# rfahrn/RadVLM

Hardware: AMD Instinct MI355X
Metric: train image-instruction pairs/sec, LLaVA-1.5-7B 336px (higher is better)
Workload: dtype bf16; 1 GPU; llava15_7b full fine-tune step (ViT frozen): fwd+bwd+AdamW, S=704, 32 pairs/GPU/step; global_batch=32, seq_len=704, parallelism=dp1, rows_with_a_label_only=last layer's o_proj / norm / MLP, final norm, lm_head, cross entropy

## Files before the change

include/radvlm_hip.h:

```cpp
#ifndef RADVLM_HIP_H
#define RADVLM_HIP_H
#include <stdint.h>

#ifdef __cplusplus
extern "C" {
#endif

#define RV_ACT_NONE 0
#define RV_ACT_QUICK_GELU 1
#define RV_ACT_GELU 2
#define RV_ACT_GELU_TANH 3

const char* rv_version(void);

int rv_gemm_nt_bf16(const void* A, int64_t lda, const void* B, int64_t ldb, void* C, int64_t ldc, const void* bias,
                    const void* residual, int64_t ldr, int M, int N, int K, int act, int out_f32, int res_f32,
                    const void* zeros16, void* stream);
int rv_gemm_bf16(const void* A, int64_t lda, const void* B, int64_t ldb, void* C, int64_t ldc, const void* bias,
                 const void* residual, int64_t ldr, int M, int N, int K, int trans_a, int trans_b, float alpha, int act,
                 int out_f32, int res_f32, const void* zeros16, void* stream);
int rv_gemm_bf16_ex(const void* A, int64_t lda, const void* B, int64_t ldb, void* C, int64_t ldc, const void* bias,
                    const void* residual, int64_t ldr, int M, int N, int K, int trans_a, int trans_b, float alpha, int act,
                    int out_f32, int res_f32, const void* A2, int64_t lda2, const void* B2, int64_t ldb2, int K2,
                    void* workspace, int64_t workspace_bytes, const void* zeros16, void* stream);
int rv_gemm_rope_bf16(const void* A, int64_t lda, const void* B, int64_t ldb, void* C, int64_t ldc, const void* bias, int M, int N, int K,
                      const float* cos_sin, const int32_t* positions, int S, int rope_heads, int hd, void* workspace,
                      int64_t workspace_bytes, const void* zeros16, void* stream);
int rv_gemm_swiglu_fwd_bf16(const void* A, int64_t lda, const void* Wgu, int64_t ldb, void* GU, int64_t ldgu, void* ACT, int64_t ldact,
                            int M, int F, int K, void* workspace, int64_t workspace_bytes, const void* zeros16, void* stream);
int rv_gemm_swiglu_bwd_bf16(const void* dY, int64_t ldy, const void* Wd, int64_t ldw, const void* GU, int64_t ldgu, void* dGU, int64_t lddgu,
                            void* dact_scratch, int64_t ld_dact, int M, int F, int K, void* workspace, int64_t workspace_bytes,
                            const void* zeros16, void* stream);
int rv_gemm_select_kernel(int which);
int rv_gemm_set_cu_budget(int total_cus, int reserved_cus);

int rv_transpose_bf16(const void* in, int64_t in_ld, int64_t in_bs0, int64_t in_bs1, void* out, int64_t out_ld,
                      int64_t out_bs0, int64_t out_bs1, int R, int C, int R_pad, int nb0, int nb1, int perm32,
                      void* stream);

int rv_rmsnorm_fwd(const void* x, const void* w, void* y, float* rstd, int rows, int d, float eps, void* stream);
int rv_rmsnorm_bwd(const void* dy, const void* x, const void* w, const float* rstd, void* dx, int dx_add,
                   float* dw_partial, int nblk, int rows, int d, void* stream);
int rv_layernorm_fwd(const void* x, const void* w, const void* b, void* y, float* stats, int rows, int d, float eps,
                     void* stream);
int rv_layernorm_bwd(const void* dy, const void* x, const void* w, const float* stats, void* dx, int dx_add,
                     float* partial, int nblk, int rows, int d, void* stream);
int rv_quick_gelu_fwd(const void* x, void* y, int64_t n, void* stream);
int rv_quick_gelu_bwd(const void* dy, const void* x, void* dx, int64_t n, void* stream);

int rv_gelu_tanh_fwd(const void* x, void* y, int64_t n, void* stream);
int rv_gelu_tanh_bwd(const void* dy, const void* x, void* dx, int64_t n, void* stream);

int rv_colsum_f32(const float* in, int rows, int cols, void* out_bf16, int accumulate, void* stream);
int rv_colsum_partial_bf16(const void* x, int64_t ld, int rows, int cols, float* partial, int nblk, void* stream);

int rv_rope_inplace(void* x, int64_t ld, const float* cos_sin, int rows, int S, int heads, int hd, int nsec, int dir,
                    void* stream);

int rv_attn_fwd(const void* q, int64_t ld_q, const void* k, int64_t ld_k, const void* vT, void* out, int64_t ld_o,
                float* lse, const int32_t* lens, int B, int H, int S, int S_pad, int hd, int causal, float scale,
                const void* zeros16, void* stream);
int rv_attn_bwd(const void* q, int64_t ld_q, const void* k, int64_t ld_k, const void* v, int64_t ld_v, const void* o,
                int64_t ld_o, const void* dout, int64_t ld_do, const void* qT, const void* kT, const void* doT,
                const float* lse, float* delta, void* dq, int64_t ld_dq, void* dk, int64_t ld_dk, void* dv,
                int64_t ld_dv, const int32_t* lens, int B, int H, int S, int S_pad, int hd, int causal, float scale,
                const void* zeros16, void* stream);

int rv_attn_fwd_gqa(const void* q, int64_t ld_q, const void* k, int64_t ld_k, const void* vT, void* out, int64_t ld_o,
                    float* lse, const int32_t* lens, const int32_t* cu_rows, int B, int H, int H_kv, int S, int S_pad, int hd,
                    int causal, float scale, const void* zeros16, void* stream);
int rv_attn_fwd_nat(const void* q, int64_t ld_q, const void* k, int64_t ld_k, const void* v, int64_t ld_v, void* out, int64_t ld_o,
                    float* lse, const int32_t* lens, const int32_t* cu_rows, int B, int H, int H_kv, int S, int S_pad, int hd, int causal,
                    float scale, const void* zeros16, void* stream);
int rv_attn_fwd_nat_pairs(int B, int H, int S, int causal);
int rv_attn_bwd_gqa(const void* q, int64_t ld_q, const void* k, int64_t ld_k, const void* v, int64_t ld_v, const void* o,
                    int64_t ld_o, const void* dout, int64_t ld_do, const void* qT, const void* kT, const void* doT,
                    const float* lse, float* delta, void* dq, int64_t ld_dq, void* dk, int64_t ld_dk, void* dv,
                    int64_t ld_dv, const int32_t* lens, const int32_t* cu_rows, int total_rows, int B, int H, int H_kv, int S,
                    int S_pad, int hd, int causal, float scale, void* workspace, int64_t workspace_bytes, const void* zeros16,
                    void* stream);
int rv_attn_bwd_gqa_rope(const void* q, int64_t ld_q, const void* k, int64_t ld_k, const void* v, int64_t ld_v, const void* o,
                         int64_t ld_o, const void* dout, int64_t ld_do, const void* qT, const void* kT, const void* doT,
                         const float* lse, float* delta, void* dq, int64_t ld_dq, void* dk, int64_t ld_dk, void* dv,
                         int64_t ld_dv, const int32_t* lens, const int32_t* cu_rows, int total_rows, int B, int H, int H_kv, int S,
                         int S_pad, int hd, int causal, float scale, void* workspace, int64_t workspace_bytes,
                         const float* rope_cos_sin, const int32_t* rope_positions, const void* zeros16, void* stream);

// ... 92 lines not shown
```

radvlm_amd/csrc/gemm_bf16.hip:

```cpp
#include <type_traits>
#include "common.h"
#include "radvlm_hip.h"
#include <stdlib.h>

namespace {

constexpr int BM = 128, BN = 128, BK = 64;
constexpr int STAGE_BYTES = (BM + BN) * BK * 2;
constexpr int NSTAGE = 2;

struct GemmParams {
    const bf16* A; const bf16* B; void* C; const bf16* bias; const void* R; const bf16* zeros;
    long lda, ldb, ldc, ldr;
    int M, N, K, act, out_f32, res_f32, tiles_m, tiles_n;
    float alpha;
    const bf16* A2; const bf16* B2; long lda2, ldb2; int K2;
    float* ws; int splits;
    int n_full;
    int pgrid;
    const float* rope_cs; const int* rope_pos; int rope_S, rope_cols, rope_hd;
    int F; bf16* C2; long ldc2; const bf16* G; long ldg;
    unsigned bytesA, bytesB;
    unsigned bytesA2, bytesB2;
    unsigned drop_thr; float drop_scale; unsigned long long drop_seed;
};
enum { EPI_NONE = 0, EPI_ROPE = 1, EPI_SWIGLU_FWD = 2, EPI_SWIGLU_BWD = 3 };

DEVINL float erf_as(float x) {
    const float ax = fabsf(x);
    const float t = __frcp_rn(1.f + 0.3275911f * ax);
    const float p = t * (0.254829592f + t * (-0.284496736f + t * (1.421413741f + t * (-1.453152027f + t * 1.061405429f))));
    const float r = 1.f - p * __expf(-ax * ax);
    return copysignf(r, x);
}
DEVINL float apply_act(float x, int act) {
    if (act == RV_ACT_QUICK_GELU) return x / (1.f + __expf(-1.702f * x));
    if (act == RV_ACT_GELU) return 0.5f * x * (1.f + erf_as(x * 0.70710678118654752f));
    if (act == RV_ACT_GELU_TANH) return x / (1.f + __expf(-1.5957691216057308f * (x + 0.044715f * x * x * x)));
    return x;
}

DEVINL void stage_tile(const bf16* __restrict__ src, long ld, int row0, int nrows_total, int k0, int K,
                       const bf16* zeros, char* lds, int wid, int lane) {
#pragma unroll
    for (int it = 0; it < 4; ++it) {
        const int c = (it * 4 + wid) * 64 + lane;
        const int r = c >> 3, p = c & 7;
        const int lc = p ^ ((r >> 1) & 7);
        const int gr = row0 + r, gk = k0 + lc * 8;
        const bf16* g = (gr < nrows_total && gk < K) ? (src + (long)gr * ld + gk) : zeros;
        glds16(g, lds + (it * 4 + wid) * 1024);
    }
}

DEVINL bf16x8 read_frag(const char* tile, int row, int kchunk) {
    const int p = kchunk ^ ((row >> 1) & 7);
    return *(const bf16x8*)(tile + row * 128 + p * 16);
}

__global__ __launch_bounds__(256, 2) void gemm_nt_kernel(GemmParams P) {
    extern __shared__ __attribute__((aligned(16))) char smem[];
    const int wid = wave_id(), lane = lane_id();
    const int wr = wid >> 1, wc = wid & 1;

    const int nwg = P.tiles_m * P.tiles_n;
    int pid = xcd_remap(blockIdx.x, nwg);
    constexpr int GROUP_M = 8;
    const int per_group = GROUP_M * P.tiles_n;
    const int group = pid / per_group;
    const int first_m = group * GROUP_M;
    const int gsz = min(P.tiles_m - first_m, GROUP_M);
    const int tm = first_m + (pid % per_group) % gsz;
    const int tn = (pid % per_group) / gsz;
    const int m0 = tm * BM, n0 = tn * BN;

    f32x4 acc[4][4];
#pragma unroll
    for (int i = 0; i < 4; ++i)
#pragma unroll
// ... 591 lines not shown
            bf16x8 gq[2][4], uq[2][4];
            auto fetch = [&](int bi, bf16x8 (&gd)[4], bf16x8 (&ud)[4]) {
#pragma unroll
                for (int u = 0; u < 4; ++u) {
                    const int ia = bi * 4 + u, i = ia >> 1, a = ia & 1;
                    const bf16* p = gp + (long)i * 16 * P.ldg + 32 * a;
                    gd[u] = *(const bf16x8*)p;
                    ud[u] = *(const bf16x8*)(p + P.F);
                }
            };
            fetch(0, gq[0], uq[0]);
            static_for<4>([&](auto bt) {
                constexpr int bi = decltype(bt)::value;
                if constexpr (bi + 1 < 4) fetch(bi + 1, gq[(bi + 1) & 1], uq[(bi + 1) & 1]);
                static_for<4>([&](auto ut) {
                    constexpr int u = decltype(ut)::value, ia = bi * 4 + u, i = ia >> 1, a = ia & 1;
                    bf16* c = cp + (long)i * 16 * P.ldc + 32 * a;
                    dswiglu(acc[i][2 * a], acc[i][2 * a + 1], gq[bi & 1][u], uq[bi & 1][u], c, c + P.F);
                });
            });
            return;
        }
        static_for<16>([&](auto ia) {
            constexpr int i = decltype(ia)::value >> 1, a = decltype(ia)::value & 1;
            const int m = m0 + wr * 128 + i * 16 + (lane & 15);
            const int n = tn * BN2 + wc * 64 + 32 * a + 8 * q;
            if (m >= P.M || n >= P.F) return;
            const bf16x8 gv = *(const bf16x8*)(P.G + (long)m * P.ldg + n), uv = *(const bf16x8*)(P.G + (long)m * P.ldg + P.F + n);
            bf16* cp = (bf16*)P.C + (long)m * P.ldc;
            dswiglu(acc[i][2 * a], acc[i][2 * a + 1], gv, uv, cp + n, cp + P.F + n);
        });
    }
}

#ifdef RV_STAMPS
static long long* g_stamp_host = nullptr;
extern "C" int rv_debug_set_stamp_buffer(void* p) { g_stamp_host = (long long*)p; return 0; }
#define RV_STAMP(i) do { if (MODE == 0 && P.ws && threadIdx.x == 0) ((long long*)P.ws)[(long)blockIdx.x * 4 + (i)] = wall_clock64(); } while (0)
#else
#define RV_STAMP(i) do { } while (0)
#endif

template <bool TA, bool TB, int MODE, int EPI = EPI_NONE, bool BUF = false>
__global__ __launch_bounds__(512, 1) void gemm_kernel_256(GemmParams P) {
    extern __shared__ __attribute__((aligned(16))) char smem[];
    const int wid = wave_id(), lane = lane_id();
    const int wr = wid >> 2, wc = wid & 3;
    RV_STAMP(0);

    const int nwg = P.tiles_m * P.tiles_n;
    constexpr bool PERSIST = (MODE == 0 || MODE == 1 || MODE == 3) && BUF;
    int vtile = blockIdx.x, kslice = 0;
    bool sliced = MODE == 2;
    if (MODE == 2) { vtile = (int)blockIdx.x / P.splits; kslice = (int)blockIdx.x % P.splits; }
    if (MODE == 3 && (int)blockIdx.x >= (PERSIST ? P.pgrid : P.n_full)) {
        const int r = (int)blockIdx.x - (PERSIST ? P.pgrid : P.n_full);
        vtile = P.n_full + r / P.splits; kslice = r % P.splits; sliced = true;
    }
    int m0, n0, tn;
    auto coords = [&](int vt) {
        const int pid = xcd_remap(vt, nwg);
        constexpr int GROUP_M = RV_GROUP_M;
        const int per_group = GROUP_M * P.tiles_n;
        const int group = pid / per_group;
        const int first_m = group * GROUP_M;
        const int gsz = min(P.tiles_m - first_m, GROUP_M);
        tn = (pid % per_group) / gsz;
        m0 = (first_m + (pid % per_group) % gsz) * BM2;
        n0 = tn * BN2;
    };
    coords(vtile);

    f32x4 acc[8][4];

    const int nt1 = (P.K + BK - 1) / BK;
    const int t0 = sliced ? (int)((long)kslice * nt1 / P.splits) : 0;
    const int nt = sliced ? (int)((long)(kslice + 1) * nt1 / P.splits) - t0 : (MODE == 1 ? nt1 + (P.K2 + BK - 1) / BK : nt1);
    __amdgpu_buffer_rsrc_t rsA, rsB;
    HalfPlan plA[2], plB[2];
    if constexpr (BUF) {
        rsA = __builtin_amdgcn_make_buffer_rsrc((void*)P.A, 0, P.bytesA, 0x00020000);
        rsB = __builtin_amdgcn_make_buffer_rsrc((void*)P.B, 0, P.bytesB, 0x00020000);
    }
    auto make_plans = [&]() {
#pragma unroll
        for (int h = 0; h < 2; ++h) {
            plA[h] = plan_half<TA, false, 0>(P.lda, m0 + h * 128, P.M, wid, lane, h, 0, P.bytesA);
            if (EPI == EPI_ROPE) plB[h] = P.rope_hd == 128 ? plan_half<TB, true, 1>(P.ldb, n0 + h * 128, P.N, wid, lane, h, 0, P.bytesB)
                                                            : plan_half<TB, true, 0>(P.ldb, n0 + h * 128, P.N, wid, lane, h, 0, P.bytesB);
            else if (EPI == EPI_SWIGLU_FWD) plB[h] = plan_half<TB, true, 2>(P.ldb, tn * 128, P.N, wid, lane, h, P.F, P.bytesB);
            else plB[h] = plan_half<TB, true, 0>(P.ldb, n0 + h * 128, P.N, wid, lane, h, 0, P.bytesB);
        }
    };
    __amdgpu_buffer_rsrc_t rsA2, rsB2;
    HalfPlan plA2[2], plB2[2];
    if constexpr (BUF && MODE == 1) {
        rsA2 = __builtin_amdgcn_make_buffer_rsrc((void*)P.A2, 0, P.bytesA2, 0x00020000);
        rsB2 = __builtin_amdgcn_make_buffer_rsrc((void*)P.B2, 0, P.bytesB2, 0x00020000);
    }
    auto make_plans2 = [&]() {
#pragma unroll
        for (int h = 0; h < 2; ++h) {
            plA2[h] = plan_half<TA, false, 0>(P.lda2, m0 + h * 128, P.M, wid, lane, h, 0, P.bytesA2);
            plB2[h] = plan_half<TB, true, 0>(P.ldb2, n0 + h * 128, P.N, wid, lane, h, 0, P.bytesB2);
        }
    };
    if constexpr (BUF) make_plans();
    if constexpr (BUF && MODE == 1) make_plans2();
    const int kstepA = TA ? (int)(P.lda * BK * 2) : BK * 2, kstepB = TB ? (int)(P.ldb * BK * 2) : BK * 2;
    const int kstepA2 = TA ? (int)(P.lda2 * BK * 2) : BK * 2, kstepB2 = TB ? (int)(P.ldb2 * BK * 2) : BK * 2;
    auto stageA = [&](int t, int slot, int h, auto pair_tag) {
        constexpr int PAIR = decltype(pair_tag)::value;
        char* dst = smem + (slot * 2 + h) * HALF_BYTES;
        if constexpr (BUF) {
            if (MODE == 1 && (PAIR == 1 || (PAIR == 2 && t >= nt1))) stage_half_buf(rsA2, plA2[h], (t - nt1) * kstepA2, dst, wid);
            else stage_half_buf(rsA, plA[h], (t0 + t) * kstepA, dst, wid);
            return;
        }
        if (MODE == 1 && t >= nt1) stage_half<TA>(P.A2, P.lda2, m0 + h * 128, P.M, (t - nt1) * BK, P.K2, P.zeros, dst, wid, lane);
        else stage_half<TA>(P.A, P.lda, m0 + h * 128, P.M, (t0 + t) * BK, P.K, P.zeros, dst, wid, lane);
    };
    auto stageB = [&](int t, int h, auto pair_tag) {
        constexpr int PAIR = decltype(pair_tag)::value;
        char* dst = smem + B_RING_OFF + ((t & 1) * 2 + h) * HALF_BYTES;
        if constexpr (BUF) {
            if (MODE == 1 && (PAIR == 1 || (PAIR == 2 && t >= nt1))) stage_half_buf(rsB2, plB2[h], (t - nt1) * kstepB2, dst, wid);
            else stage_half_buf(rsB, plB[h], (t0 + t) * kstepB, dst, wid);
            return;
        }
        if (MODE == 1 && t >= nt1) stage_half<TB, true>(P.B2, P.ldb2, n0 + h * 128, P.N, (t - nt1) * BK, P.K2, P.zeros, dst, wid, lane);
// ... 11 lines not shown
    int vt0 = blockIdx.x;
    do {
    if (nt > 1) { stageA(1, 1, 0, PR); stageA(1, 1, 1, PR); stageB(1, 0, PR); stageB(1, 1, PR); asm volatile("s_waitcnt vmcnt(8)" ::: "memory"); }
    else asm volatile("s_waitcnt vmcnt(0)" ::: "memory");
    __builtin_amdgcn_s_barrier();
    RV_STAMP(1);
#pragma unroll
    for (int i = 0; i < 8; ++i)
#pragma unroll
        for (int j = 0; j < 4; ++j) acc[i][j] = f32x4{0.f, 0.f, 0.f, 0.f};

    int aslot = 0;
    long long dbg[4] = {0, 0, 0, 0};
    auto step = [&](int t, auto stage_tag, auto pair_tag) {
        constexpr int STAGE = decltype(stage_tag)::value;
        const char* At = smem + (aslot * 2 + wr) * HALF_BYTES;
        const char* Bt = smem + B_RING_OFF + ((t & 1) * 2 + (wc >> 1)) * HALF_BYTES;
        const int aslot2 = aslot == 0 ? 2 : aslot - 1;
        const int brow0 = (wc & 1) * 64;
        ktile_256<TA, TB>(acc, At, Bt, brow0, lane,
                          [&]() { if (STAGE == 1 || (STAGE == 2 && t + 2 < nt)) stageA(t + 2, aslot2, 0, pair_tag); },
                          [&]() { if (STAGE == 1 || (STAGE == 2 && t + 2 < nt)) stageA(t + 2, aslot2, 1, pair_tag); },
                          [&]() { if (STAGE == 1 || (STAGE == 2 && t + 2 < nt)) stageB(t + 2, 0, pair_tag); },
                          [&]() { if (STAGE == 1 || (STAGE == 2 && t + 2 < nt)) stageB(t + 2, 1, pair_tag); }, dbg);
        RV_ACC_BEGIN();
        if (STAGE == 1 || (STAGE == 2 && t + 2 < nt)) asm volatile("s_waitcnt vmcnt(8)" ::: "memory");
        else asm volatile("s_waitcnt vmcnt(0)" ::: "memory");
        RV_ACC_END(1);
        aslot = aslot == 2 ? 0 : aslot + 1;
        RV_ACC_BEGIN();
        BAR_LGKM();
        RV_ACC_END(2);
    };
    if constexpr ((MODE == 2 || MODE == 1) && !BUF) {
        for (int t = 0; t < nt; ++t) step(t, std::integral_constant<int, 2>{}, PR);
    } else if constexpr (MODE == 1) {
        int t = 0;
        for (; t + 2 < nt1; ++t) step(t, std::integral_constant<int, 1>{}, P0);
        for (; t + 2 < nt; ++t) step(t, std::integral_constant<int, 1>{}, P1);
        for (; t < nt; ++t) step(t, std::integral_constant<int, 0>{}, P0);
    } else {
        int t = 0;
        for (; t + 2 < nt; ++t) step(t, std::integral_constant<int, 1>{}, P0);
        for (; t < nt; ++t) step(t, std::integral_constant<int, 0>{}, P0);
    }
#ifdef RV_STAMPS
    if (MODE == 0 && P.ws && lane == 0) {
        long long* o = (long long*)P.ws + (long)gridDim.x * 4 + ((long)blockIdx.x * 8 + wid) * 3;
        o[0] = dbg[0]; o[1] = dbg[1]; o[2] = dbg[2];
    }
#endif

    RV_STAMP(2);
    if (MODE == 3 && sliced) {
        float* slab = P.ws + ((long)(vtile - P.n_full) * P.splits + kslice) * (BM2 * BN2);
#pragma unroll
        for (int i = 0; i < 8; ++i)
#pragma unroll
            for (int a = 0; a < 2; ++a) {
                float* wp = slab + (wr * 128 + i * 16 + (lane & 15)) * BN2 + wc * 64 + 32 * a + 8 * (lane >> 4);
                *(f32x4*)wp = acc[i][2 * a];
                *(f32x4*)(wp + 4) = acc[i][2 * a + 1];
            }
        return;
    }
    const int m0e = m0, n0e = n0, tne = tn;
    bool more = false;
    if constexpr (PERSIST) {
        vt0 += MODE == 3 ? P.pgrid : (int)gridDim.x;
        more = !sliced && vt0 < (MODE == 3 ? P.n_full : nwg);
        if (more) {
            coords(vt0); make_plans();
            if constexpr (MODE == 1) make_plans2();
            stageA(0, 0, 0, P0); stageA(0, 0, 1, P0); stageB(0, 0, P0); stageB(0, 1, P0);
        }
    }
    if (EPI != EPI_NONE) epilogue_fused<EPI>(acc, P, m0e, tne, wr, wc, lane);
    else epilogue_256<MODE == 3 ? 0 : MODE>(acc, P, m0e, n0e, wr, wc, lane, kslice);
#ifdef RV_STAMPS
    asm volatile("s_waitcnt vmcnt(0)" ::: "memory");
#endif
    RV_STAMP(3);
    if (!more) break;
    } while (PERSIST);
}

__global__ void splitk_reduce_kernel(GemmParams P) {
    const long i = (long)blockIdx.x * blockDim.x + threadIdx.x;
    const long total = (long)P.M * P.N;
    if (i >= total) return;
    const int m = (int)(i / P.N), n = (int)(i % P.N);
    float s = 0.f;
    for (int k = 0; k < P.splits; ++k) s += P.ws[(long)k * total + i];
    s *= P.alpha;
    if (P.bias) s += bf2f(P.bias[n]);
    s = apply_act(s, P.act);
    if (P.R) s += P.res_f32 ? ((const float*)P.R)[(long)m * P.ldr + n] : bf2f(((const bf16*)P.R)[(long)m * P.ldr + n]);
    if (P.out_f32) ((float*)P.C)[(long)m * P.ldc + n] = s;
    else ((bf16*)P.C)[(long)m * P.ldc + n] = f2bf(s);
}

constexpr int AG_BM = 64, AG_BN = 128;
constexpr int AG_XB = AG_BM * AG_BN * 2, AG_TB = AG_BM * 64 * 2, AG_STAGE = AG_XB + AG_TB;
struct LoraAGradParams {
    const bf16* X; const bf16* T; float* ws;
    long ldx, ldt;
    int M, R, K, splits;
    unsigned thr; unsigned long long seed;
};
DEVINL int sw128(int m) { return (((m >> 1) & 1) | (((m >> 3) & 1) << 1)) << 1; }
DEVINL bf16x8 tr_read16(const char* a, const char* b) {
    const s16x4 lo = __builtin_amdgcn_ds_read_tr16_b64_v4i16((__attribute__((address_space(3))) s16x4*)a);
    const s16x4 hi = __builtin_amdgcn_ds_read_tr16_b64_v4i16((__attribute__((address_space(3))) s16x4*)b);
    const s16x8 r = {lo[0], lo[1], lo[2], lo[3], hi[0], hi[1], hi[2], hi[3]};
    return __builtin_bit_cast(bf16x8, r);
}
__global__ __launch_bounds__(256, 3) void lora_agrad_kernel(LoraAGradParams P) {
    __shared__ __attribute__((aligned(16))) char smem[2 * AG_STAGE];
    const int wid = wave_id(), lane = lane_id(), tid = (int)threadIdx.x;
    const int ncb = (P.K + AG_BN - 1) / AG_BN;
    const int cb = (int)blockIdx.x % ncb, split = (int)blockIdx.x / ncb;
// ... 34 lines not shown
#pragma unroll
    for (int i = 0; i < 4; ++i) toff[i] = AG_XB + mrow * 128 + ((((16 * i) >> 3) + (pp >> 1)) ^ sw128(mrow)) * 16 + (pp & 1) * 8;
    f32x4 acc[4][2];
#pragma unroll
    for (int i = 0; i < 4; ++i)
#pragma unroll
        for (int j = 0; j < 2; ++j) acc[i][j] = f32x4{0.f, 0.f, 0.f, 0.f};
    if (s0 < s1) { load(s0); store(s0, smem); }
    __syncthreads();
    for (int s = s0; s < s1; ++s) {
        const char* cur = smem + ((s - s0) & 1) * AG_STAGE;
        char* nxt = smem + (((s - s0) & 1) ^ 1) * AG_STAGE;
        if (s + 1 < s1) load(s + 1);
#pragma unroll
        for (int kk = 0; kk < 2; ++kk) {
            bf16x8 b[2], a[4];
#pragma unroll
            for (int j = 0; j < 2; ++j) b[j] = tr_read16(cur + xoff[j] + kk * 8192, cur + xoff[j] + kk * 8192 + 1024);
#pragma unroll
            for (int i = 0; i < 4; ++i) a[i] = tr_read16(cur + toff[i] + kk * 4096, cur + toff[i] + kk * 4096 + 512);
#pragma unroll
            for (int i = 0; i < 4; ++i)
#pragma unroll
                for (int j = 0; j < 2; ++j) acc[i][j] = mfma16(a[i], b[j], acc[i][j]);
        }
        if (s + 1 < s1) store(s + 1, nxt);
        __syncthreads();
    }
#pragma unroll
    for (int i = 0; i < 4; ++i)
#pragma unroll
        for (int j = 0; j < 2; ++j)
#pragma unroll
            for (int r = 0; r < 4; ++r) {
                const int ar = 16 * i + 4 * g + r, col = c0 + wid * 32 + 16 * j + (lane & 15);
                if (ar < P.R && col < P.K) P.ws[((long)split * P.R + ar) * P.K + col] = acc[i][j][r];
            }
}

__global__ __launch_bounds__(256) void tail_reduce_kernel(GemmParams P) {
    const int nwg = P.tiles_m * P.tiles_n;
    const int tt = blockIdx.x >> 5;
    const int e = ((blockIdx.x & 31) * 256 + threadIdx.x) * 8;
    const int row = e >> 8, col = e & 255;
    const int pid = xcd_remap(P.n_full + tt, nwg);
    constexpr int GROUP_M = RV_GROUP_M;
    const int per_group = GROUP_M * P.tiles_n;
    const int group = pid / per_group;
    const int first_m = group * GROUP_M;
    const int gsz = min(P.tiles_m - first_m, GROUP_M);
    const int m = (first_m + (pid % per_group) % gsz) * BM2 + row;
    const int n = ((pid % per_group) / gsz) * BN2 + col;
    if (m >= P.M || n >= P.N) return;
    float v[8] = {0, 0, 0, 0, 0, 0, 0, 0};
    for (int k = 0; k < P.splits; ++k) {
        const float* sp = P.ws + ((long)tt * P.splits + k) * (BM2 * BN2) + row * BN2 + col;
        const f32x4 a = *(const f32x4*)sp, b = *(const f32x4*)(sp + 4);
#pragma unroll
        for (int r = 0; r < 4; ++r) { v[r] += a[r]; v[4 + r] += b[r]; }
    }
    const int nv = min(8, P.N - n);
    const bool vec = nv == 8 && (P.N % 8 == 0) && (P.ldc % 8 == 0) && !P.out_f32 && (!P.R || (!P.res_f32 && P.ldr % 8 == 0)) &&
                     ((((uintptr_t)P.C) | ((uintptr_t)P.R) | ((uintptr_t)P.bias)) & 15) == 0;
    if (vec) {
        float x[8];
#pragma unroll
        for (int r = 0; r < 8; ++r) x[r] = v[r] * P.alpha;
        if (P.bias) {
            const bf16x8 bb = *(const bf16x8*)(P.bias + n);
#pragma unroll
            for (int r = 0; r < 8; ++r) x[r] += bf2f(bb[r]);
        }
        if (P.act != RV_ACT_NONE) {
#pragma unroll
            for (int r = 0; r < 8; ++r) x[r] = apply_act(x[r], P.act);
        }
        if (P.R) {
            const bf16x8 rr = *(const bf16x8*)((const bf16*)P.R + (long)m * P.ldr + n);
#pragma unroll
            for (int r = 0; r < 8; ++r) x[r] += bf2f(rr[r]);
        }
        *(bf16x8*)((bf16*)P.C + (long)m * P.ldc + n) = bf16x8{f2bf(x[0]), f2bf(x[1]), f2bf(x[2]), f2bf(x[3]), f2bf(x[4]), f2bf(x[5]), f2bf(x[6]), f2bf(x[7])};
        return;
    }
    for (int r = 0; r < nv; ++r) {
        float x = v[r] * P.alpha;
        if (P.bias) x += bf2f(P.bias[n + r]);
        x = apply_act(x, P.act);
        if (P.R) x += P.res_f32 ? ((const float*)P.R)[(long)m * P.ldr + n + r] : bf2f(((const bf16*)P.R)[(long)m * P.ldr + n + r]);
        if (P.out_f32) ((float*)P.C)[(long)m * P.ldc + n + r] = x;
        else ((bf16*)P.C)[(long)m * P.ldc + n + r] = f2bf(x);
    }
}

}

static int g_tail_split = 1;
static int g_force_kernel = 0;
static int g_cus = 0;
static int g_cus_device = -1;
static int g_reserved_cus = -1;
static int g_no_buf = 0;
static int g_persist = 1;
extern "C" int rv_gemm_select_kernel(int which) {
    if (which >= 40) { g_persist = which == 41; return RV_OK; }
    if (which >= 30) { g_no_buf = which == 30; return RV_OK; }
    if (which >= 20) { g_tail_split = which - 20; return RV_OK; }
    g_force_kernel = which;
    return RV_OK;
}
extern "C" int rv_gemm_set_cu_budget(int total_cus, int reserved_cus) {
    int dev = 0;
    if (hipGetDevice(&dev) != hipSuccess) return RV_ERR_LAUNCH;
    if (total_cus <= 0) {
        int n = 0;
        if (hipDeviceGetAttribute(&n, hipDeviceAttributeMultiprocessorCount, dev) != hipSuccess) return RV_ERR_LAUNCH;
        total_cus = n;
    }
    g_cus_device = dev;
    if (reserved_cus < 0) reserved_cus = 0;
    g_reserved_cus = reserved_cus;
    g_cus = total_cus - reserved_cus;
    if (g_cus < 8) g_cus = 8;
    return g_cus;
}
static int cu_budget() {
    int dev = 0;
    if (g_cus != 0 && hipGetDevice(&dev) == hipSuccess && dev != g_cus_device) g_cus = 0;
    if (g_cus == 0) {
        const char* e = getenv("RV_GEMM_RESERVED_CUS");
        rv_gemm_set_cu_budget(0, g_reserved_cus >= 0 ? g_reserved_cus : (e ? atoi(e) : 0));
    }
    return g_cus;
}

static bool buf_extents(GemmParams& P, int trans_a, int trans_b) {
    if ((P.K % BK) && !(trans_a && trans_b)) return false;
    const long ea = (trans_a ? (long)P.K : (long)P.M) * P.lda * 2, eb = (trans_b ? (long)P.K : (long)P.N) * P.ldb * 2;
    if (ea >= (1L << 31) || eb >= (1L << 31) || g_no_buf) return false;
    P.bytesA = (unsigned)ea; P.bytesB = (unsigned)eb;
    return true;
}
static bool buf_extents2(GemmParams& P, int trans_a, int trans_b) {
    if ((P.K2 % BK) && !(trans_a && trans_b)) return false;
    const long ea = (trans_a ? (long)P.K2 : (long)P.M) * P.lda2 * 2, eb = (trans_b ? (long)P.K2 : (long)P.N) * P.ldb2 * 2;
    if (ea >= (1L << 31) || eb >= (1L << 31)) return false;
    P.bytesA2 = (unsigned)ea; P.bytesB2 = (unsigned)eb;
    return true;
}
template <bool TA, bool TB, int MODE, bool BUF = false>
static void launch256m(const GemmParams& P, hipStream_t st) {
    static bool set = false;
    if (!set) { (void)hipFuncSetAttribute((const void*)gemm_kernel_256<TA, TB, MODE, EPI_NONE, BUF>, hipFuncAttributeMaxDynamicSharedMemorySize, LDS_BYTES2); set = true; }
    const int nwg = P.tiles_m * P.tiles_n;
    const int blocks = MODE == 2 ? nwg * P.splits : (MODE == 3 ? P.n_full + (nwg - P.n_full) * P.splits : nwg);
    int grid = blocks;
    GemmParams Q = P;
    Q.pgrid = MODE == 3 ? P.n_full : blocks;
    if (g_persist && BUF && (MODE == 0 || MODE == 1) && blocks > cu_budget()) { grid = cu_budget(); Q.pgrid = grid; }
    if (g_persist && BUF && MODE == 3 && P.n_full > cu_budget()) { Q.pgrid = cu_budget(); grid = Q.pgrid + (nwg - P.n_full) * P.splits; }
    hipLaunchKernelGGL((gemm_kernel_256<TA, TB, MODE, EPI_NONE, BUF>), dim3(grid), dim3(512), LDS_BYTES2, st, Q);
    if (MODE == 3) hipLaunchKernelGGL(tail_reduce_kernel, dim3((nwg - P.n_full) * 32), dim3(256), 0, st, P);
    if (MODE == 2) {
        const long total = (long)P.M * P.N;
        hipLaunchKernelGGL(splitk_reduce_kernel, dim3((unsigned)((total + 255) / 256)), dim3(256), 0, st, P);
    }
}
template <bool TA, bool TB>
static void launch256(GemmParams& P, int mode, hipStream_t st) {
    if (mode == 1) { if (buf_extents(P, TA, TB) && buf_extents2(P, TA, TB)) launch256m<TA, TB, 1, true>(P, st); else launch256m<TA, TB, 1>(P, st); }
    else if (mode == 2) { if (buf_extents(P, TA, TB)) launch256m<TA, TB, 2, true>(P, st); else launch256m<TA, TB, 2>(P, st); }
    else if (buf_extents(P, TA, TB)) { if (mode == 3) launch256m<TA, TB, 3, true>(P, st); else launch256m<TA, TB, 0, true>(P, st); }
    else if (mode == 3) launch256m<TA, TB, 3>(P, st);
    else launch256m<TA, TB, 0>(P, st);
}

static int gemm_ex_impl(const void* A, int64_t lda, const void* B, int64_t ldb, void* C, int64_t ldc, const void* bias,
                        const void* residual, int64_t ldr, int M, int N, int K, int trans_a, int trans_b, float alpha,
                        int act, int out_f32, int res_f32, const void* A2, int64_t lda2, const void* B2, int64_t ldb2,
                        int K2, void* workspace, int64_t workspace_bytes, const void* zeros16, void* stream, float drop_p, uint64_t drop_seed) {
    if (!A || !B || !C || !zeros16 || M <= 0 || N <= 0 || K <= 0) return RV_ERR_ARG;
    if ((lda & 7) || (ldb & 7)) return RV_ERR_ARG;
    if ((!trans_a && (K & 7)) || (trans_a && (M & 7)) || (!trans_b && (K & 7)) || (trans_b && (N & 7))) return RV_ERR_ARG;
    if (((uintptr_t)A | (uintptr_t)B | (uintptr_t)zeros16) & 15) return RV_ERR_ARG;
    const bool ext = A2 && B2 && K2 > 0;
    if (ext && ((lda2 & 7) || (ldb2 & 7) || (!trans_a && (K2 & 7)) || (!trans_b && (K2 & 7)) || (((uintptr_t)A2 | (uintptr_t)B2) & 15))) return RV_ERR_ARG;
    GemmParams P;
    P.A = (const bf16*)A; P.B = (const bf16*)B; P.C = C; P.bias = (const bf16*)bias; P.R = residual;
    P.zeros = (const bf16*)zeros16;
    P.lda = lda; P.ldb = ldb; P.ldc = ldc; P.ldr = ldr;
    P.M = M; P.N = N; P.K = K; P.act = act; P.out_f32 = out_f32; P.res_f32 = res_f32; P.alpha = alpha;
    P.A2 = (const bf16*)A2; P.B2 = (const bf16*)B2; P.lda2 = lda2; P.ldb2 = ldb2; P.K2 = ext ? K2 : 0;
    P.ws = (float*)workspace; P.splits = 1;
    P.drop_thr = drop_p > 0.f ? rv_dropout_thr16(drop_p) : 0u; P.drop_scale = drop_p > 0.f ? 1.f / (1.f - drop_p) : 1.f; P.drop_seed = drop_seed;
    const bool dropping = P.drop_thr != 0;
    static bool attr_set = false;
    if (!attr_set) {
        (void)hipFuncSetAttribute((const void*)gemm_nt_kernel, hipFuncAttributeMaxDynamicSharedMemorySize, NSTAGE * STAGE_BYTES);
        const char* e = getenv("RV_GEMM_KERNEL");
        if (e) g_force_kernel = atoi(e);
        attr_set = true;
    }
    const long tiles256 = (long)((M + BM2 - 1) / BM2) * ((N + BN2 - 1) / BN2);
    const int nt = (K + BK - 1) / BK;
    const int force = g_force_kernel;
    const int cus = cu_budget();
    int mode = ext ? 1 : 0;
    if (dropping) workspace = nullptr;
    if (!ext && workspace && tiles256 <= cus / 4 && nt >= 16) {
        int sp = (int)(cus / tiles256);
        if (sp > nt / 4) sp = nt / 4;
        if (sp > 32) sp = 32;
        if (sp >= 2 && (int64_t)sp * M * N * 4 <= workspace_bytes) { mode = 2; P.splits = sp; }
    }
    P.n_full = 0;
    if (mode == 0 && workspace && g_tail_split && tiles256 > cus) {
        const int rem = (int)(tiles256 % cus);
        if (rem > 0 && rem <= cus / 2 && nt >= 32) {
            int sp = cus / rem;
            if (sp > 4) sp = 4;
            if ((int64_t)rem * sp * BM2 * BN2 * 4 <= workspace_bytes) { mode = 3; P.splits = sp; P.n_full = (int)(tiles256 - rem); }
        }
    }
    const long tiles128 = (long)((M + BM - 1) / BM) * ((N + BN - 1) / BN);
    const double cost256 = 4.0 * (double)((tiles256 + cus - 1) / cus);
    const double cost128 = 2.0 * 1.15 * (double)((tiles128 + 2 * cus - 1) / (2 * cus));
    const bool use256 = (trans_a || trans_b || mode || dropping) ? true : (force ? (force == 2) : (cost256 <= cost128));
    hipStream_t st = (hipStream_t)stream;
    if (use256) {
#ifdef RV_STAMPS
        if (mode == 0) P.ws = (float*)g_stamp_host;
#endif
        P.tiles_m = (M + BM2 - 1) / BM2; P.tiles_n = (N + BN2 - 1) / BN2;
        if (trans_a) { if (trans_b) launch256<true, true>(P, mode, st); else launch256<true, false>(P, mode, st); }
        else { if (trans_b) launch256<false, true>(P, mode, st); else launch256<false, false>(P, mode, st); }
    } else {
        P.tiles_m = (M + BM - 1) / BM; P.tiles_n = (N + BN - 1) / BN;
        hipLaunchKernelGGL(gemm_nt_kernel, dim3(P.tiles_m * P.tiles_n), dim3(256), NSTAGE * STAGE_BYTES, st, P);
    }
    return rv_check_launch();
}

extern "C" int rv_gemm_bf16_ex(const void* A, int64_t lda, const void* B, int64_t ldb, void* C, int64_t ldc, const void* bias,
                               const void* residual, int64_t ldr, int M, int N, int K, int trans_a, int trans_b, float alpha,
                               int act, int out_f32, int res_f32, const void* A2, int64_t lda2, const void* B2, int64_t ldb2,
                               int K2, void* workspace, int64_t workspace_bytes, const void* zeros16, void* stream) {
    return gemm_ex_impl(A, lda, B, ldb, C, ldc, bias, residual, ldr, M, N, K, trans_a, trans_b, alpha, act, out_f32, res_f32, A2, lda2, B2, ldb2, K2,
                        workspace, workspace_bytes, zeros16, stream, 0.f, 0);
}

extern "C" int rv_gemm_dropout_add_bf16(const void* A, int64_t lda, const void* B, int64_t ldb, void* C, int64_t ldc, int M, int N, int K,
                                        int trans_b, float alpha, float p, uint64_t seed, int accumulate, const void* zeros16, void* stream) {
    if (p < 0.f || p >= 1.f || (N & 7) || (ldc & 7) || (((uintptr_t)C) & 15)) return RV_ERR_ARG;
    return gemm_ex_impl(A, lda, B, ldb, C, ldc, nullptr, accumulate ? C : nullptr, ldc, M, N, K, 0, trans_b, alpha, RV_ACT_NONE, 0, 0, nullptr, 0,
                        nullptr, 0, 0, nullptr, 0, zeros16, stream, p, seed);
}

extern "C" int rv_gemm_bf16(const void* A, int64_t lda, const void* B, int64_t ldb, void* C, int64_t ldc, const void* bias,
                            const void* residual, int64_t ldr, int M, int N, int K, int trans_a, int trans_b, float alpha,
                            int act, int out_f32, int res_f32, const void* zeros16, void* stream) {
    return rv_gemm_bf16_ex(A, lda, B, ldb, C, ldc, bias, residual, ldr, M, N, K, trans_a, trans_b, alpha, act, out_f32, res_f32,
                           nullptr, 0, nullptr, 0, 0, nullptr, 0, zeros16, stream);
}

extern "C" int rv_gemm_nt_bf16(const void* A, int64_t lda, const void* B, int64_t ldb, void* C, int64_t ldc,
                               const void* bias, const void* residual, int64_t ldr, int M, int N, int K, int act,
                               int out_f32, int res_f32, const void* zeros16, void* stream) {
    return rv_gemm_bf16(A, lda, B, ldb, C, ldc, bias, residual, ldr, M, N, K, 0, 0, 1.0f, act, out_f32, res_f32, zeros16, stream);
}

template <int EPI, bool TB, bool BUF>
static void launch_fused1(const GemmParams& P, hipStream_t st) {
    static bool attr = false;
    if (!attr) { (void)hipFuncSetAttribute((const void*)gemm_kernel_256<false, TB, 0, EPI, BUF>, hipFuncAttributeMaxDynamicSharedMemorySize, LDS_BYTES2); attr = true; }
    int grid = P.tiles_m * P.tiles_n;
// ... 123 lines not shown
```

radvlm_amd/lib.py:

```python
import ctypes
import os

import torch

_HERE = os.path.dirname(os.path.abspath(__file__))
_LIB_PATH = os.path.join(_HERE, "libradvlm_hip.so")

_c_void_p = ctypes.c_void_p
_i64 = ctypes.c_int64
_i32 = ctypes.c_int
_f32 = ctypes.c_float

ACT_NONE, ACT_QUICK_GELU, ACT_GELU, ACT_GELU_TANH = 0, 1, 2, 3

_SIGS = {
    "rv_gemm_nt_bf16": [_c_void_p, _i64, _c_void_p, _i64, _c_void_p, _i64, _c_void_p, _c_void_p, _i64, _i32, _i32, _i32,
                        _i32, _i32, _i32, _c_void_p, _c_void_p],
    "rv_gemm_bf16": [_c_void_p, _i64, _c_void_p, _i64, _c_void_p, _i64, _c_void_p, _c_void_p, _i64, _i32, _i32, _i32, _i32, _i32,
                     _f32, _i32, _i32, _i32, _c_void_p, _c_void_p],
    "rv_gemm_bf16_ex": [_c_void_p, _i64, _c_void_p, _i64, _c_void_p, _i64, _c_void_p, _c_void_p, _i64, _i32, _i32, _i32, _i32, _i32,
                        _f32, _i32, _i32, _i32, _c_void_p, _i64, _c_void_p, _i64, _i32, _c_void_p, _i64, _c_void_p, _c_void_p],
    "rv_gemm_rope_bf16": [_c_void_p, _i64, _c_void_p, _i64, _c_void_p, _i64, _c_void_p, _i32, _i32, _i32, _c_void_p, _c_void_p, _i32, _i32, _i32,
                          _c_void_p, _i64, _c_void_p, _c_void_p],
    "rv_gemm_swiglu_fwd_bf16": [_c_void_p, _i64, _c_void_p, _i64, _c_void_p, _i64, _c_void_p, _i64, _i32, _i32, _i32, _c_void_p, _i64, _c_void_p,
# ... 32 lines not shown
                        _c_void_p, _i64, _c_void_p, _i64, _c_void_p, _c_void_p, _i32, _i32, _i32, _i32, _i32, _i32, _i32, _i32, _f32, _c_void_p, _i64,
                        _c_void_p, _c_void_p, _c_void_p, _c_void_p],
    "rv_attn_bwd_gqa_rope": [_c_void_p, _i64, _c_void_p, _i64, _c_void_p, _i64, _c_void_p, _i64, _c_void_p, _i64, _c_void_p, _c_void_p,
                             _c_void_p, _c_void_p, _c_void_p, _c_void_p, _i64, _c_void_p, _i64, _c_void_p, _i64, _c_void_p, _c_void_p, _i32,
                             _i32, _i32, _i32, _i32, _i32, _i32, _i32, _f32, _c_void_p, _i64, _c_void_p, _c_void_p, _c_void_p, _c_void_p],
    "rv_transpose_bf16_varlen": [_c_void_p, _i64, _c_void_p, _i64, _c_void_p, _i64, _i64, _i64, _i32, _i32, _i32, _i32, _i32, _i32,
                                 _c_void_p],
    "rv_rope_inplace_pos": [_c_void_p, _i64, _c_void_p, _c_void_p, _i32, _i32, _i32, _i32, _i32, _c_void_p],
    "rv_gelu_tanh_fwd": [_c_void_p, _c_void_p, _i64, _c_void_p],
    "rv_gelu_tanh_bwd": [_c_void_p, _c_void_p, _c_void_p, _i64, _c_void_p],
    "rv_weighted_segment_sum_rows": [_c_void_p, _i64, _c_void_p, _c_void_p, _c_void_p, _c_void_p, _i32, _c_void_p, _i64, _i32,
                                     _c_void_p],
    "rv_max4_rows_fwd": [_c_void_p, _i64, _c_void_p, _c_void_p, _i32, _c_void_p, _i64, _c_void_p, _i32, _c_void_p],
    "rv_max4_rows_bwd": [_c_void_p, _i64, _c_void_p, _c_void_p, _i32, _c_void_p, _c_void_p, _i64, _i32, _c_void_p],
    "rv_add_pos_rows": [_c_void_p, _c_void_p, _i32, _i32, _i32, _c_void_p],
    "rv_swiglu_fwd": [_c_void_p, _i64, _c_void_p, _i64, _i32, _i32, _c_void_p],
    "rv_swiglu_bwd": [_c_void_p, _i64, _c_void_p, _i64, _c_void_p, _i64, _i32, _i32, _c_void_p],
    "rv_gelu_fwd": [_c_void_p, _c_void_p, _i64, _c_void_p],
    "rv_gelu_bwd": [_c_void_p, _c_void_p, _c_void_p, _i64, _c_void_p],
    "rv_cross_entropy": [_c_void_p, _i64, _c_void_p, _c_void_p, _c_void_p, _i64, _i32, _i32, _f32, _c_void_p],
    "rv_sum_f32": [_c_void_p, _i64, _f32, _c_void_p, _c_void_p],
    "rv_gather_rows": [_c_void_p, _i64, _c_void_p, _i64, _c_void_p, _i64, _c_void_p, _i32, _i32, _c_void_p],
    "rv_segment_sum_rows": [_c_void_p, _i64, _c_void_p, _c_void_p, _c_void_p, _i32, _c_void_p, _i64, _i32, _c_void_p],
    "rv_normalize_tiles_u8": [_c_void_p, _c_void_p, _i32, _i32, _i32, _i32, _i32, ctypes.c_double, ctypes.POINTER(_f32), ctypes.POINTER(_f32), _c_void_p],
    "rv_im2col_patches": [_c_void_p, _c_void_p, _i32, _i32, _i32, _i32, _i32, _c_void_p],
    "rv_clip_embed": [_c_void_p, _c_void_p, _c_void_p, _c_void_p, _i32, _i32, _i32, _c_void_p],
    "rv_adamw": [_c_void_p, _c_void_p, _c_void_p, _c_void_p, _c_void_p, _i64, _f32, _f32, _f32, _f32, _f32, _f32, _f32,
                 _c_void_p, _c_void_p],
    "rv_sumsq_partial_bf16": [_c_void_p, _i64, _c_void_p, _i32, _c_void_p],
    "rv_clip_coef": [_c_void_p, _i32, _f32, _c_void_p, _c_void_p],
    "rv_cast_f32_to_bf16": [_c_void_p, _c_void_p, _i64, _c_void_p],
    "rv_cast_bf16_to_f32": [_c_void_p, _c_void_p, _i64, _c_void_p],
    "rv_add_bf16": [_c_void_p, _c_void_p, _c_void_p, _i64, _c_void_p],
    "rv_gemv_bf16": [_c_void_p, _i64, _c_void_p, _i64, _c_void_p, _i64, _c_void_p, _c_void_p, _i64, _i32, _i32, _i32, _i32, _c_void_p, _i64,
                     _c_void_p],
    "rv_quantize_rows_w8_bf16": [_c_void_p, _i64, _c_void_p, _i64, _c_void_p, _i32, _i32, _c_void_p],
    "rv_gemv_w8_bf16": [_c_void_p, _i64, _c_void_p, _i64, _c_void_p, _c_void_p, _i64, _c_void_p, _c_void_p, _i64, _i32, _i32, _i32, _i32,
                        _c_void_p, _i64, _c_void_p],
    "rv_attn_decode_bf16": [_c_void_p, _i64, _c_void_p, _i64, _i64, _i32, _c_void_p, _i32, _c_void_p, _i64, _c_void_p, _i64, _i32, _i32, _i32,
                            _i32, _i32, _f32, _c_void_p],
    "rv_attn_extend_bf16": [_c_void_p, _i64, _c_void_p, _i64, _i64, _i32, _c_void_p, _c_void_p, _i32, _c_void_p, _i64, _c_void_p, _i64, _i32,
                            _i32, _i32, _i32, _i32, _i32, _i32, _f32, _c_void_p],
    "rv_kv_append_bf16": [_c_void_p, _i64, _c_void_p, _i64, _i64, _c_void_p, _i32, _i32, _i32, _c_void_p],
    "rv_argmax_rows_f32": [_c_void_p, _i64, _i32, _i32, _c_void_p, _c_void_p],
    "rv_logits_process_argmax_f32": [_c_void_p, _i64, _i32, _i32, _c_void_p, _i64, _i32, _f32, _i32, _c_void_p, _i32, _c_void_p, _c_void_p, _i32,
                                     _c_void_p, _c_void_p],
    "rv_logits_process_argmax_rows_f32": [_c_void_p, _i64, _i32, _i32, _c_void_p, _i64, _i32, _i32, _c_void_p, _c_void_p, _c_void_p, _f32,
                                          _i32, _c_void_p, _i32, _c_void_p, _i32, _c_void_p, _i32, _c_void_p, _c_void_p, _i32, _c_void_p,
                                          _c_void_p, _c_void_p],
    "rv_lora_merge_bf16": [_c_void_p, _i64, _c_void_p, _i64, _c_void_p, _i64, _i32, _i32, _i32, _f32, _c_void_p],
}

EXPORTED_SYMBOLS = ["rv_version", "rv_gemm_select_kernel", "rv_gemm_set_cu_budget", "rv_attn_fwd_nat_pairs", "rv_gemv_split",
                    "rv_w8_row_bytes"] + sorted(_SIGS)

_lib = None


class RadvlmHipError(RuntimeError):
    pass


def load():
    global _lib
    if _lib is None:
        path = os.environ.get("RADVLM_HIP_LIB", _LIB_PATH)
        if not os.path.exists(path):
            raise RadvlmHipError(f"{path} not found: build it with radvlm_amd/csrc/build.sh "
                                 "(or __graft_entry__.build()); there is no CPU fallback")
        lib = ctypes.CDLL(path)
        lib.rv_version.restype = ctypes.c_char_p
        lib.rv_w8_row_bytes.argtypes = [_i32]
        lib.rv_w8_row_bytes.restype = _i64
        for name, sig in _SIGS.items():
            fn = getattr(lib, name)
            fn.argtypes = sig
            fn.restype = _i32
        _lib = lib
    return _lib


def _ptr(t):
    if t is None:
        return None
    if isinstance(t, int):
        return t
    assert t.is_cuda, "radvlm_amd kernels take device tensors only"
    return t.data_ptr()


def _stream():
    return torch.cuda.current_stream().cuda_stream


def call(name, *args):
    lib = load()
    rc = getattr(lib, name)(*[(_ptr(a) if (a is None or isinstance(a, torch.Tensor)) else a) for a in args], _stream())
    if rc != 0:
        raise RadvlmHipError(f"{name} failed with code {rc}")


_zeros = {}


def zeros16(device=None):
    device = torch.device(device or torch.cuda.current_device())
    key = (device.type, device.index)
    if key not in _zeros:
        _zeros[key] = torch.zeros(64, dtype=torch.uint8, device=device)
    return _zeros[key]
```

Baseline: 43.60 pairs/s.

## Split GEMM tail tiles into balanced stream-K shares across CUs

Replaces the fixed per-tile K-split of the last partial wave with a stream-K style partition. The leftover tiles' K iterations are cut into S roughly equal shares (one per CU), and a share may cross a tile boundary. The reduce kernel now sums over the variable shares that cover each tile. A cost heuristic chooses between this even split and the old fixed split, and it can also apply when the tile count is below the CU count. The goal is a smaller wave-quantization tail on large GEMMs, at the cost of extra workspace traffic, a reduction pass and more complex indexing. Host-side plan query functions are exported for inspection.

After: 43.40 pairs/s. Within noise of the previous version (-0.5%).

```diff
diff --git a/include/radvlm_hip.h b/include/radvlm_hip.h
--- a/include/radvlm_hip.h
+++ b/include/radvlm_hip.h
@@ -33,6 +33,8 @@
                             const void* zeros16, void* stream);
 int rv_gemm_select_kernel(int which);
 int rv_gemm_set_cu_budget(int total_cus, int reserved_cus);
+int rv_gemm_plan_query(int M, int N, int K, int cus, int64_t workspace_bytes, int32_t* out8);
+int rv_gemm_plan_share(int M, int N, int K, int cus, int64_t workspace_bytes, int share, int32_t* out8);
 
 int rv_transpose_bf16(const void* in, int64_t in_ld, int64_t in_bs0, int64_t in_bs1, void* out, int64_t out_ld,
                       int64_t out_bs0, int64_t out_bs1, int R, int C, int R_pad, int nb0, int nb1, int perm32,
diff --git a/radvlm_amd/csrc/gemm_bf16.hip b/radvlm_amd/csrc/gemm_bf16.hip
--- a/radvlm_amd/csrc/gemm_bf16.hip
+++ b/radvlm_amd/csrc/gemm_bf16.hip
@@ -16,7 +16,7 @@
     float alpha;
     const bf16* A2; const bf16* B2; long lda2, ldb2; int K2;
     float* ws; int splits;
-    int n_full;
+    int n_full, shares, slab_tt;
     int pgrid;
     const float* rope_cs; const int* rope_pos; int rope_S, rope_cols, rope_hd;
     int F; bf16* C2; long ldc2; const bf16* G; long ldg;
@@ -25,6 +25,16 @@
     unsigned drop_thr; float drop_scale; unsigned long long drop_seed;
 };
 enum { EPI_NONE = 0, EPI_ROPE = 1, EPI_SWIGLU_FWD = 2, EPI_SWIGLU_BWD = 3 };
+
+constexpr int TAIL_MIN_PIECE = 4;
+constexpr int TAIL_MIN_SHARE = 8;
+__host__ __device__ inline long tail_bound(long j, long W, int S, int nt) {
+    long b = j * W / S;
+    const int r = (int)(b % nt);
+    if (r < TAIL_MIN_PIECE) b -= r;
+    else if (nt - r < TAIL_MIN_PIECE) b -= r - (nt - TAIL_MIN_PIECE);
+    return b;
+}
 
 DEVINL float erf_as(float x) {
     const float ax = fabsf(x);
@@ -722,10 +732,31 @@
     constexpr bool PERSIST = (MODE == 0 || MODE == 1 || MODE == 3) && BUF;
     int vtile = blockIdx.x, kslice = 0;
     bool sliced = MODE == 2;
-    if (MODE == 2) { vtile = (int)blockIdx.x / P.splits; kslice = (int)blockIdx.x % P.splits; }
+    const int nt1 = (P.K + BK - 1) / BK;
+    int t0 = 0, nt = MODE == 1 ? nt1 + (P.K2 + BK - 1) / BK : nt1, rest = 0, slab_id = 0;
+    if (MODE == 2) {
+        vtile = (int)blockIdx.x / P.splits; kslice = (int)blockIdx.x % P.splits;
+        t0 = (int)((long)kslice * nt1 / P.splits);
+        nt = (int)((long)(kslice + 1) * nt1 / P.splits) - t0;
+    }
     if (MODE == 3 && (int)blockIdx.x >= (PERSIST ? P.pgrid : P.n_full)) {
         const int r = (int)blockIdx.x - (PERSIST ? P.pgrid : P.n_full);
-        vtile = P.n_full + r / P.splits; kslice = r % P.splits; sliced = true;
+        const int j = BUF ? r : r >> 1;
+        const long W = (long)(nwg - P.n_full) * nt1;
+        const long ua = tail_bound(j, W, P.shares, nt1), ub = tail_bound(j + 1, W, P.shares, nt1);
+        if (ua >= ub) return;
+        const int tt = (int)(ua / nt1);
+        vtile = P.n_full + tt; sliced = true; slab_id = j + P.slab_tt * tt;
+        t0 = (int)(ua - (long)tt * nt1);
+        nt = (int)min(ub - ua, (long)(nt1 - t0));
+        rest = (int)(ub - ua) - nt;
+        if (!BUF) {
+            if (r & 1) {
+                if (!rest) return;
+                ++vtile; slab_id += P.slab_tt; t0 = 0; nt = rest;
+            }
+            rest = 0;
+        }
     }
     int m0, n0, tn;
     auto coords = [&](int vt) {
@@ -743,9 +774,6 @@
 
     f32x4 acc[8][4];
 
-    const int nt1 = (P.K + BK - 1) / BK;
-    const int t0 = sliced ? (int)((long)kslice * nt1 / P.splits) : 0;
-    const int nt = sliced ? (int)((long)(kslice + 1) * nt1 / P.splits) - t0 : (MODE == 1 ? nt1 + (P.K2 + BK - 1) / BK : nt1);
     __amdgpu_buffer_rsrc_t rsA, rsB;
     HalfPlan plA[2], plB[2];
     if constexpr (BUF) {
@@ -863,21 +891,29 @@
 #endif
 
     RV_STAMP(2);
-    if (MODE == 3 && sliced) {
-        float* slab = P.ws + ((long)(vtile - P.n_full) * P.splits + kslice) * (BM2 * BN2);
-#pragma unroll
-        for (int i = 0; i < 8; ++i)
-#pragma unroll
-            for (int a = 0; a < 2; ++a) {
-                float* wp = slab + (wr * 128 + i * 16 + (lane & 15)) * BN2 + wc * 64 + 32 * a + 8 * (lane >> 4);
-                *(f32x4*)wp = acc[i][2 * a];
-                *(f32x4*)(wp + 4) = acc[i][2 * a + 1];
-            }
-        return;
-    }
     const int m0e = m0, n0e = n0, tne = tn;
     bool more = false;
-    if constexpr (PERSIST) {
+    if (MODE == 3 && sliced) {
+        const bool whole = t0 == 0 && nt == nt1;
+        float* slab = P.ws + (long)slab_id * (BM2 * BN2);
+        if constexpr (BUF) if (rest) {
+            ++vtile; slab_id += P.slab_tt; t0 = 0; nt = rest; rest = 0; more = true;
+            coords(vtile); make_plans();
+            stageA(0, 0, 0, P0); stageA(0, 0, 1, P0); stageB(0, 0, P0); stageB(0, 1, P0);
+        }
+        if (!whole) {
+#pragma unroll
+            for (int i = 0; i < 8; ++i)
+#pragma unroll
+                for (int a = 0; a < 2; ++a) {
+                    float* wp = slab + (wr * 128 + i * 16 + (lane & 15)) * BN2 + wc * 64 + 32 * a + 8 * (lane >> 4);
+                    *(f32x4*)wp = acc[i][2 * a];
+                    *(f32x4*)(wp + 4) = acc[i][2 * a + 1];
+                }
+            if (!more) break;
+            continue;
+        }
+    } else if constexpr (PERSIST) {
         vt0 += MODE == 3 ? P.pgrid : (int)gridDim.x;
         more = !sliced && vt0 < (MODE == 3 ? P.n_full : nwg);
         if (more) {
@@ -1018,9 +1054,14 @@
     const int m = (first_m + (pid % per_group) % gsz) * BM2 + row;
     const int n = ((pid % per_group) / gsz) * BN2 + col;
     if (m >= P.M || n >= P.N) return;
+    const int nt = (P.K + BK - 1) / BK;
+    const long W = (long)(nwg - P.n_full) * nt, u0 = (long)tt * nt, u1 = u0 + nt;
+    int j = (int)(u0 * P.shares / W);
+    while (tail_bound(j + 1, W, P.shares, nt) <= u0) ++j;
+    if (tail_bound(j + 1, W, P.shares, nt) >= u1) return;
     float v[8] = {0, 0, 0, 0, 0, 0, 0, 0};
-    for (int k = 0; k < P.splits; ++k) {
-        const float* sp = P.ws + ((long)tt * P.splits + k) * (BM2 * BN2) + row * BN2 + col;
+    for (; j < P.shares && tail_bound(j, W, P.shares, nt) < u1; ++j) {
+        const float* sp = P.ws + (long)(j + P.slab_tt * tt) * (BM2 * BN2) + row * BN2 + col;
         const f32x4 a = *(const f32x4*)sp, b = *(const f32x4*)(sp + 4);
 #pragma unroll
         for (int r = 0; r < 4; ++r) { v[r] += a[r]; v[4 + r] += b[r]; }
@@ -1119,12 +1160,12 @@
     static bool set = false;
     if (!set) { (void)hipFuncSetAttribute((const void*)gemm_kernel_256<TA, TB, MODE, EPI_NONE, BUF>, hipFuncAttributeMaxDynamicSharedMemorySize, LDS_BYTES2); set = true; }
     const int nwg = P.tiles_m * P.tiles_n;
-    const int blocks = MODE == 2 ? nwg * P.splits : (MODE == 3 ? P.n_full + (nwg - P.n_full) * P.splits : nwg);
+    const int blocks = MODE == 2 ? nwg * P.splits : (MODE == 3 ? P.n_full + (BUF ? 1 : 2) * P.shares : nwg);
     int grid = blocks;
     GemmParams Q = P;
     Q.pgrid = MODE == 3 ? P.n_full : blocks;
     if (g_persist && BUF && (MODE == 0 || MODE == 1) && blocks > cu_budget()) { grid = cu_budget(); Q.pgrid = grid; }
-    if (g_persist && BUF && MODE == 3 && P.n_full > cu_budget()) { Q.pgrid = cu_budget(); grid = Q.pgrid + (nwg - P.n_full) * P.splits; }
+    if (g_persist && BUF && MODE == 3 && P.n_full > cu_budget()) { Q.pgrid = cu_budget(); grid = Q.pgrid + P.shares; }
     hipLaunchKernelGGL((gemm_kernel_256<TA, TB, MODE, EPI_NONE, BUF>), dim3(grid), dim3(512), LDS_BYTES2, st, Q);
     if (MODE == 3) hipLaunchKernelGGL(tail_reduce_kernel, dim3((nwg - P.n_full) * 32), dim3(256), 0, st, P);
     if (MODE == 2) {
@@ -1139,6 +1180,59 @@
     else if (buf_extents(P, TA, TB)) { if (mode == 3) launch256m<TA, TB, 3, true>(P, st); else launch256m<TA, TB, 0, true>(P, st); }
     else if (mode == 3) launch256m<TA, TB, 3>(P, st);
     else launch256m<TA, TB, 0>(P, st);
+}
+
+struct GemmPlan { int mode, splits, n_full, tail, shares, slab_tt, slabs, nt; };
+constexpr int EVEN_FIXED_STEPS = 8;
+constexpr double EVEN_SLAB_STEPS = 0.07;
+static GemmPlan plan_gemm(int M, int N, int K, int cus, int64_t ws_bytes, bool tail_split) {
+    GemmPlan pl = {0, 1, 0, 0, 0, 0, 0, (K + BK - 1) / BK};
+    const long tiles = (long)((M + BM2 - 1) / BM2) * ((N + BN2 - 1) / BN2);
+    const int nt = pl.nt;
+    const int64_t slab_bytes = (int64_t)BM2 * BN2 * 4;
+    if (ws_bytes > 0 && tiles <= cus / 4 && nt >= 16) {
+        int sp = (int)(cus / tiles);
+        if (sp > nt / 4) sp = nt / 4;
+        if (sp > 32) sp = 32;
+        if (sp >= 2 && (int64_t)sp * M * N * 4 <= ws_bytes) { pl.mode = 2; pl.splits = sp; return pl; }
+    }
+    if (!tail_split || ws_bytes <= 0 || nt < 32) return pl;
+    const int rem = tiles > cus ? (int)(tiles % cus) : (tiles > cus / 4 && tiles < cus ? (int)tiles : 0);
+    if (rem == 0) return pl;
+    const long W = (long)rem * nt;
+    const int S = (int)(W / TAIL_MIN_SHARE < cus ? W / TAIL_MIN_SHARE : cus);
+    const double saved = (double)nt - (double)W / S;
+    if (S > rem && (int64_t)(S + rem) * slab_bytes <= ws_bytes && saved >= EVEN_FIXED_STEPS + EVEN_SLAB_STEPS * (S + rem)) {
+        pl.mode = 3; pl.n_full = (int)(tiles - rem); pl.tail = rem; pl.shares = S; pl.slab_tt = 1; pl.slabs = S + rem;
+        return pl;
+    }
+    if (tiles > cus && rem <= cus / 2) {
+        int sp = cus / rem;
+        if (sp > 4) sp = 4;
+        if ((int64_t)rem * sp * slab_bytes <= ws_bytes) {
+            pl.mode = 3; pl.n_full = (int)(tiles - rem); pl.tail = rem; pl.shares = rem * sp; pl.slab_tt = 0; pl.slabs = rem * sp;
+        }
+    }
+    return pl;
+}
+extern "C" int rv_gemm_plan_query(int M, int N, int K, int cus, int64_t workspace_bytes, int32_t* out8) {
+    if (M <= 0 || N <= 0 || K <= 0 || cus < 1 || !out8) return RV_ERR_ARG;
+    const GemmPlan pl = plan_gemm(M, N, K, cus, workspace_bytes, g_tail_split != 0);
+    const int o[8] = {pl.mode, pl.splits, pl.n_full, pl.tail, pl.shares, pl.nt, TAIL_MIN_PIECE, pl.slabs};
+    for (int i = 0; i < 8; ++i) out8[i] = o[i];
+    return RV_OK;
+}
+extern "C" int rv_gemm_plan_share(int M, int N, int K, int cus, int64_t workspace_bytes, int share, int32_t* out8) {
+    if (M <= 0 || N <= 0 || K <= 0 || cus < 1 || !out8) return RV_ERR_ARG;
+    const GemmPlan pl = plan_gemm(M, N, K, cus, workspace_bytes, g_tail_split != 0);
+    if (pl.mode != 3 || share < 0 || share >= pl.shares) return RV_ERR_ARG;
+    const long W = (long)pl.tail * pl.nt;
+    const long ua = tail_bound(share, W, pl.shares, pl.nt), ub = tail_bound(share + 1, W, pl.shares, pl.nt);
+    const int tt = (int)(ua / pl.nt), t0 = (int)(ua - (long)tt * pl.nt);
+    const int len = (int)(ub - ua < pl.nt - t0 ? ub - ua : pl.nt - t0), rest = (int)(ub - ua) - len;
+    const int o[8] = {(ub > ua) + (rest > 0), tt, t0, len, share + pl.slab_tt * tt, tt + 1, rest, share + pl.slab_tt * (tt + 1)};
+    for (int i = 0; i < 8; ++i) out8[i] = o[i];
+    return RV_OK;
 }
 
 static int gemm_ex_impl(const void* A, int64_t lda, const void* B, int64_t ldb, void* C, int64_t ldc, const void* bias,
@@ -1171,22 +1265,12 @@
     const int nt = (K + BK - 1) / BK;
     const int force = g_force_kernel;
     const int cus = cu_budget();
-    int mode = ext ? 1 : 0;
     if (dropping) workspace = nullptr;
-    if (!ext && workspace && tiles256 <= cus / 4 && nt >= 16) {
-        int sp = (int)(cus / tiles256);
-        if (sp > nt / 4) sp = nt / 4;
-        if (sp > 32) sp = 32;
-        if (sp >= 2 && (int64_t)sp * M * N * 4 <= workspace_bytes) { mode = 2; P.splits = sp; }
-    }
-    P.n_full = 0;
-    if (mode == 0 && workspace && g_tail_split && tiles256 > cus) {
-        const int rem = (int)(tiles256 % cus);
-        if (rem > 0 && rem <= cus / 2 && nt >= 32) {
-            int sp = cus / rem;
-            if (sp > 4) sp = 4;
-            if ((int64_t)rem * sp * BM2 * BN2 * 4 <= workspace_bytes) { mode = 3; P.splits = sp; P.n_full = (int)(tiles256 - rem); }
-        }
+    int mode = 1;
+    P.n_full = 0; P.shares = 0; P.slab_tt = 0;
+    if (!ext) {
+        const GemmPlan pl = plan_gemm(M, N, K, cus, workspace ? workspace_bytes : 0, g_tail_split != 0);
+        mode = pl.mode; P.splits = pl.splits; P.n_full = pl.n_full; P.shares = pl.shares; P.slab_tt = pl.slab_tt;
     }
     const long tiles128 = (long)((M + BM - 1) / BM) * ((N + BN - 1) / BN);
     const double cost256 = 4.0 * (double)((tiles256 + cus - 1) / cus);
diff --git a/radvlm_amd/lib.py b/radvlm_amd/lib.py
--- a/radvlm_amd/lib.py
+++ b/radvlm_amd/lib.py
@@ -108,7 +108,7 @@
 }
 
 EXPORTED_SYMBOLS = ["rv_version", "rv_gemm_select_kernel", "rv_gemm_set_cu_budget", "rv_attn_fwd_nat_pairs", "rv_gemv_split",
-                    "rv_w8_row_bytes"] + sorted(_SIGS)
+                    "rv_w8_row_bytes", "rv_gemm_plan_query", "rv_gemm_plan_share"] + sorted(_SIGS)
 
 _lib = None
 
@@ -128,6 +128,9 @@
         lib.rv_version.restype = ctypes.c_char_p
         lib.rv_w8_row_bytes.argtypes = [_i32]
         lib.rv_w8_row_bytes.restype = _i64
+        if "RADVLM_HIP_LIB" not in os.environ or hasattr(lib, "rv_gemm_plan_query"):
+            lib.rv_gemm_plan_query.argtypes = [_i32, _i32, _i32, _i32, _i64, ctypes.POINTER(ctypes.c_int32)]
+            lib.rv_gemm_plan_share.argtypes = [_i32, _i32, _i32, _i32, _i64, _i32, ctypes.POINTER(ctypes.c_int32)]
         for name, sig in _SIGS.items():
             fn = getattr(lib, name)
             fn.argtypes = sig
```
